# zj15001/PNP_ADMM_CNC_MRI

Measured on AMD Instinct MI355X. Metric: ADMM iterations/sec on 256x256 complex64 slices (batch=512), higher is better.
Workload: dtype f32

## Files before the change

### pnp_admm_cnc_mri_amd/csrc/api.hip

```cpp
#include "../../include/pnp_mri.h"
#include "internal.h"
#include "wavelet_plan.h"
#include "coil_plan.h"
#include "coilmix_plan.h"
#include "coilmaps_plan.h"

#include <math.h>
#include <stdarg.h>
#include <stdio.h>
#include <stdlib.h>
#include <string.h>
#include <dlfcn.h>
#include <new>
#include <type_traits>
#include <vector>

using namespace pnp;

static thread_local char g_err[512] = "";

int pnp::fail(int code, const char* fmt, ...) {
    va_list ap;
    va_start(ap, fmt);
    vsnprintf(g_err, sizeof(g_err), fmt, ap);
// ... 204 lines not shown
        if (c->mask_bank) { HIPCHK(hipStreamSynchronize(c->stream)); HIPCHK(hipFree(c->mask_bank)); c->mask_bank = nullptr; c->Kcap = 0; }
        HIPCHK(hipMalloc((void**)&c->mask_bank, (size_t)K * c->N));
        c->Kcap = K;
    }
    int rc = copy_in(c, c->mask_bank, mask_bank, (size_t)K * c->N, on_device);
    if (rc) return rc;
    if (mask_id) {
        std::vector<int32_t> tmp;
        const int32_t* ids = mask_id;
        if (on_device) {
            tmp.resize((size_t)B);
            HIPCHK(hipMemcpyAsync(tmp.data(), mask_id, (size_t)B * sizeof(int32_t), hipMemcpyDeviceToHost, c->stream));
            HIPCHK(hipStreamSynchronize(c->stream));
            ids = tmp.data();
        }
        for (int i = 0; i < B; ++i) if (ids[i] < 0 || ids[i] >= K) return fail(PNP_E_ARG, "mask_id[%d]=%d out of range [0,%d)", i, ids[i], K);
        rc = copy_in(c, c->mask_id, mask_id, (size_t)B * sizeof(int32_t), on_device);
        if (rc) return rc;
    } else {
        HIPCHK(hipMemsetAsync(c->mask_id, 0, (size_t)B * sizeof(int32_t), c->stream));
    }
    c->B = B; c->K = K;
    return PNP_OK;
}

static bool slice_pays(const pnp_ctx* c) { return c->B >= c->eng.slice_min_b; }

static int ensure_tables(pnp_ctx* c, Path path) {
    const float2* y = (const float2*)c->y;
    switch (path) {
    case Path::generic:
        return PNP_OK;
    case Path::slice:
        if (!c->prob.slice_built) HIPCHK(slice256_prepare(c->eng.slice, c->stream, y, c->mask_bank, c->mask_id, c->B));
        c->prob.slice_built = true;
        return PNP_OK;
    case Path::fused:
        if (c->prob.fused_built) return PNP_OK;
        switch (c->eng.kind) {
        case Engine::none:      return PNP_OK;
        case Engine::fused256:  HIPCHK(fused256_prepare(c->eng.f256, c->stream, y, c->mask_bank, c->mask_id, c->B)); break;
        case Engine::split_f32: HIPCHK(fused256s_prepare<float>(c->eng.s32, c->stream, c->y, c->mask_bank, c->mask_id, c->B)); break;
        case Engine::split_f64: HIPCHK(fused256s_prepare<double>(c->eng.s64, c->stream, c->y, c->mask_bank, c->mask_id, c->B)); break;
        case Engine::fused512:  HIPCHK(fused512_prepare(c->eng.f512, c->stream, y, c->mask_bank, c->mask_id, c->B)); break;
        }
        c->prob.fused_built = true;
        return PNP_OK;
    }
    return PNP_OK;
}

static int finish_problem(pnp_ctx* c, int rc) {
    if (rc == PNP_OK && c->eng.kind != Engine::none && c->coils.C == 0) {
        c->prob.path = (c->eng.slice && slice_pays(c)) ? Path::slice : Path::fused;
        if (c->prob.path == Path::fused) rc = ensure_tables(c, Path::fused);
    }
    if (rc != PNP_OK) { c->B = 0; c->prob = Problem{}; }
    return rc;
}

static Path loop_path(const pnp_ctx* c) { return (c->fast && c->coils.C == 0) ? c->prob.path : Path::generic; }
static Path dc_path(const pnp_ctx* c) { return loop_path(c) == Path::generic ? Path::generic : Path::fused; }

template <typename R> static int state_order(pnp_ctx* c, bool sliced) {
    if constexpr (std::is_same_v<R, double>) {
        return PNP_OK;
    } else {
// ... 1464 lines not shown
```

### pnp_admm_cnc_mri_amd/csrc/internal.h

```cpp
#pragma once
#include <hip/hip_runtime.h>
#include <stdint.h>
#include <stdlib.h>
#include "loop_schedule.h"
#include "prox_params.h"
#include "trace_plan.h"

namespace pnp {

int fail(int code, const char* fmt, ...) __attribute__((format(printf, 2, 3)));
#define HIPCHK(expr)                                                                               \
    do {                                                                                           \
        hipError_t _e = (expr);                                                                    \
        if (_e != hipSuccess)                                                                      \
            return fail(PNP_E_HIP, "%s failed: %s (%s:%d)", #expr, hipGetErrorString(_e), __FILE__, __LINE__); \
    } while (0)

template <typename R> struct CxOf;
template <> struct CxOf<float>  { using type = float2; };
template <> struct CxOf<double> { using type = double2; };

enum RowIn  { IN_COMPLEX = 0, IN_REAL = 1, IN_REAL_DIFF = 2 };
enum RowEpi { EPI_COMPLEX = 0, EPI_ABS_REAL = 1, EPI_ABS_COMPLEX = 2, EPI_L1 = 3, EPI_CNC = 4 };
enum ColMid { MID_NONE = 0, MID_BLEND = 1, MID_MASK = 2, MID_RESID = 3, MID_MASK_ADD = 4 };
// ... 135 lines not shown
hipError_t launch_conv3x3_tail_f16(hipStream_t s, const void* x_nhwc, const void* x2_nhwc , const float* w_oihw,
                                   const float* bias, float* y, int n, int cout, int H, int W, int shuffle_h = 0, int shuffle_w = 0);
hipError_t launch_pix2_pack_w_f16(hipStream_t s, const float* w, void* wfrag , int C, int up);
hipError_t launch_pix2x2_f16(hipStream_t s, const void* x, const void* x2, const void* wfrag, void* y, int n, int C, int H, int W, int up, int y_f32);

enum class ChainStep { open, cols, mid, last };

struct Fused256;
Fused256*  fused256_create(int Bmax, hipError_t* err);
void       fused256_destroy(Fused256*);
hipError_t fused256_prepare(Fused256*, hipStream_t s, const float2* y, const uint8_t* mask_bank,
                            const int32_t* mask_id, int B);
hipError_t fused256_run(Fused256*, hipStream_t s, float* z, float* w, float* x, int B, int iters,
                        bool cnc, float dc_c, ProxParams p, const FusedSchedule& sch);
hipError_t fused256_dc(Fused256*, hipStream_t s, const float* z, const float* w, float* x, int B, float dc_c);
hipError_t fused256_step(Fused256*, hipStream_t s, ChainStep st, const float* z, const float* w, float* zo, float* wo, float* x, int B,
                         bool cnc, float dc_c, ProxParams p, const FusedSchedule& sch, bool u_first);

template <typename R> struct Fused256S;
template <typename R> Fused256S<R>* fused256s_create(int Bmax, hipError_t* err);
template <typename R> void          fused256s_destroy(Fused256S<R>*);
template <typename R> hipError_t    fused256s_prepare(Fused256S<R>*, hipStream_t s, const void* y, const uint8_t* mask_bank,
                                                      const int32_t* mask_id, int B);
template <typename R> hipError_t    fused256s_run(Fused256S<R>*, hipStream_t s, R* z, R* w, R* x, int B, int iters, bool cnc,
                                                  R dc_c, ProxParamsT<R> p, const FusedSchedule& sch);
template <typename R> hipError_t    fused256s_dc(Fused256S<R>*, hipStream_t s, const R* z, const R* w, R* x, int B, R dc_c);
template <typename R> hipError_t    fused256s_step(Fused256S<R>*, hipStream_t s, ChainStep st, const R* z, const R* w, R* zo, R* wo, R* x, int B,
                                                   bool cnc, R dc_c, ProxParamsT<R> p, const FusedSchedule& sch, bool u_first);

struct Slice256;
Slice256*  slice256_create(int Bmax, int pad_kb , int yh_pad_kb , hipError_t* err);
void       slice256_destroy(Slice256*);
int        slice256_cus(const Slice256*);
hipError_t slice256_prepare(Slice256*, hipStream_t s, const float2* y, const uint8_t* mask_bank, const int32_t* mask_id, int B);
hipError_t slice256_run(Slice256*, hipStream_t s, float* z, float* w, float* x, int B, int iters, bool cnc, float dc_c,
                        ProxParams p, const FusedSchedule& sch);
hipError_t slice256_state_order(Slice256*, hipStream_t s, float* z, float* w, int B, bool to_slice);
hipError_t slice256_trace_snapshot(Slice256*, hipStream_t s, const float* z, int B);
hipError_t slice256_residuals(Slice256*, hipStream_t s, const float* x, const float* z, const float* w, const uint8_t* gt, int B,
                              double* partial, unsigned* counter, double* out);

struct Fused512;
Fused512*  fused512_create(int Bmax, hipError_t* err);
void       fused512_destroy(Fused512*);
hipError_t fused512_prepare(Fused512*, hipStream_t s, const float2* y, const uint8_t* mask_bank,
                            const int32_t* mask_id, int B);
hipError_t fused512_run(Fused512*, hipStream_t s, float* z, float* w, float* x, int B, int iters,
                        bool cnc, float dc_c, ProxParams p, const FusedSchedule& sch);
hipError_t fused512_dc(Fused512*, hipStream_t s, const float* z, const float* w, float* x, int B, float dc_c);
hipError_t fused512_step(Fused512*, hipStream_t s, ChainStep st, const float* z, const float* w, float* zo, float* wo, float* x, int B,
                         bool cnc, float dc_c, ProxParams p, const FusedSchedule& sch, bool u_first);

}
```

### pnp_admm_cnc_mri_amd/csrc/kernels_slice256.hip

```cpp
#include "engine_host.h"
#include "fused_layout.h"
#include "slice_layout.h"
#include <math.h>
#include <stdio.h>
#include <stdlib.h>
#include <vector>

#ifndef SLICE_EARLY
#define SLICE_EARLY 1
#endif
#ifndef SLICE_PRIOSWAP
#define SLICE_PRIOSWAP 1
#endif
#ifndef SLICE_PRIOMASK
#define SLICE_PRIOMASK 6
#endif
#ifndef SLICE_YH_AUX
#define SLICE_YH_AUX 0
#endif
#ifndef SLICE_ST_AUX
#define SLICE_ST_AUX 0
#endif
#ifndef SLICE_PF
#define SLICE_PF 3
#endif

namespace pnp {

__device__ c32 g_tws[256];

struct SliceArgs {
    float* z;
    float* w;
    float* x;
    const c32* Yh;
    const uint32_t* Mh;
    const c32* Ys;
    const uint32_t* Ms;
    int first, B, iters;
    int slice_xor;
    int flip;
    int state_stride;
    int yh_stride;
    float scale, c;
    ProxParams prox;
    long long* prof;
};

constexpr int RP = 18;
constexpr int REGION = 16 * RP;
constexpr int WREG = 4 * REGION;
constexpr int SL_YS = SL_BUF + REGION;
constexpr int SL_LDS = SL_YS + 256 + 32;
static_assert(SL_WAVES * WREG <= SL_BUF, "wave regions must fit in the buffer they alias");
__device__ __forceinline__ int sl_lds_float(int set, int q) { return set == 0 ? sl_res_index(0, 0, q) : sl_res1_index(popc8(sl_units_lds(set) & ((1u << q) - 1)), 0, 0); }
static_assert(REGION * 8 == SL2_TW_BYTES && (256 + 32) * 8 == SL2_YS_BYTES && SL2_END % 8 == 0, "tables of the LDS map");
template <int PROX> constexpr bool slice_four() { return PROX == 2; }
template <int PROX> constexpr bool slice_res() { return slice_four<PROX>() && SLICE_RESIDENT; }
__device__ __forceinline__ void lds_ld4(const float* p, float (&v)[4]) {
    const float4 q = *reinterpret_cast<const float4*>(p);
    v[0] = q.x; v[1] = q.y; v[2] = q.z; v[3] = q.w;
}
__device__ __forceinline__ void lds_st4(float* p, const float (&v)[4]) { *reinterpret_cast<float4*>(p) = make_float4(v[0], v[1], v[2], v[3]); }

__device__ __forceinline__ void wave_sync() {
    __builtin_amdgcn_fence(__ATOMIC_RELEASE, "wavefront");
    __builtin_amdgcn_wave_barrier();
    __builtin_amdgcn_fence(__ATOMIC_ACQUIRE, "wavefront");
#ifdef SLICE_SYNC_SCHED_BARRIER
    __builtin_amdgcn_sched_barrier(0);
#endif
// ... 265 lines not shown
    const int voff = 2048 * g + 16 * t;
    float* const resl[2] = {RES ? res_lane(res, 0, wv, lane) : nullptr, RES && SL_NLDS1 ? res_lane(res, 1, wv, lane) : nullptr};
    constexpr bool RES_LOOP = RES && HAS_INV;
    constexpr int PF = row_pf<PROX>();
    RowLoads L;
    if (PRELOADED) L = *pre;
    else issue_row_loads<PROX, HAS_INV, 0, PF, RES_LOOP>(b, L, row_set_offset(0, wv), voff, 0, 0, resl[0]);
#pragma unroll
    for (int set = 0; set < SL_SETS; ++set) {
        c32 (&a)[16] = F[set];
        prio_set(wv, set);
        const int soff = row_set_offset(set, wv);
        if (HAS_INV) {
            group_fft256<true, SPLIT>(a, twl, region, t);
        }
        if (HAS_INV && last) store_x_natural<SPLIT>(b, a, wreg, set, wv, lane);
        const int vs = voff + soff;
#pragma unroll
        for (int q = 0; q < 8; ++q) {
            const int home = RES ? w_home(set, q) : W_HBM;
            float* const rl = home == W_LDS ? resl[set] + sl_lds_float(set, q) : nullptr;
            float* const wq = wr[home == W_REG ? sl_reg_slot(set, q) : 0];
            if (q + PF < 8) issue_row_loads<PROX, HAS_INV, 0, 1, RES_LOOP>(b, L, soff, voff, q + PF, set, resl[set < 2 ? set : 0]);
            if (RES_LOOP && home != W_HBM) {
                pointwise_q<HAS_INV, PROX, HAS_FWD>(b, pc, u_first, last, a[2 * q], a[2 * q + 1], L.z[q], home == W_REG ? wr[sl_reg_slot(set, q)] : L.w[q],
                                                    vs + ROW_QSTRIDE * q, home, rl, wq);
            } else {
                if (home == W_LDS) lds_st4(rl, L.w[q]);
                if (home == W_REG) { wq[0] = L.w[q][0]; wq[1] = L.w[q][1]; wq[2] = L.w[q][2]; wq[3] = L.w[q][3]; }
                pointwise_q<HAS_INV, PROX, HAS_FWD>(b, pc, u_first, last, a[2 * q], a[2 * q + 1], L.z[q], L.w[q], vs + ROW_QSTRIDE * q);
            }
        }
        if (set + 1 < SL_SETS) issue_row_loads<PROX, HAS_INV, 0, PF, RES_LOOP>(b, L, row_set_offset(set + 1, wv), voff, 0, set + 1, resl[set + 1 < 2 ? set + 1 : 0]);
        if (HAS_FWD) {
            group_fft256<false, SPLIT>(a, twl, region, t);
        }
    }
}

__device__ __forceinline__ void resident_flush(const SliceBufs& b, float* res, const ResRegs& wr, int wv, int lane) {
#pragma unroll
    for (int set = 0; set < SL_SETS; ++set) {
        const int vs = 2048 * (lane >> 4) + 16 * (lane & 15) + row_set_offset(set, wv);
#pragma unroll
        for (int q = 0; q < 8; ++q) {
            const int home = w_home(set, q);
            if (home == W_LDS) {
                float v[4];
                lds_ld4(res_lane(res, set, wv, lane) + sl_lds_float(set, q), v);
                st4(b.w, vs + ROW_QSTRIDE * q, 0, v);
            } else if (home == W_REG) {
                st4(b.w, vs + ROW_QSTRIDE * q, 0, wr[sl_reg_slot(set, q)]);
            }
        }
    }
}

#define SL_PASS0_REGS(X, t)                                                                       \
    X(0, 0, (t)) X(1, 1, (t) + 16) X(2, 2, (t) + 32) X(3, 3, (t) + 48)                              \
    X(12, 8, ((t) ? SL_M + 64 - (t) : SL_M))                                                      \
    X(13, 13, SL_M + 48 - (t)) X(14, 14, SL_M + 32 - (t)) X(15, 15, SL_M + 16 - (t))
#define SL_PASS1_REGS(X, t)                                                                       \
    X(4, 4, (t)) X(5, 5, (t) + 16) X(6, 6, (t) + 32) X(7, 7, (t) + 48)                              \
    X(8, 12, ((t) ? SL_M + 64 - (t) : SL_M))                                                      \
    X(9, 9, SL_M + 48 - (t)) X(10, 10, SL_M + 32 - (t)) X(11, 11, SL_M + 16 - (t))

#define SL_PASS4_REGS(X, t, Q)                                                                    \
// ... 196 lines not shown
        prio_set(wv, set);
        group_fft256<false, SPLIT>(a, twl, region, t);
        if (set == 0 && wv == 0 && g == 0) {
#pragma unroll
            for (int j = 0; j < 16; ++j) region[t + 16 * j] = a[j];
            region[256 + t] = a[0];
            wave_sync();
            const uint32_t code_b = reinterpret_cast<const uint32_t*>(ysl + 256)[t];
            const c32* mirror = region + (16 - t);
            const unsigned ma[4] = {Y.code & 0x03030303u, (Y.code >> 2) & 0x03030303u, (Y.code >> 4) & 0x03030303u, (Y.code >> 6) & 0x03030303u};
            const unsigned mb[4] = {code_b & 0x03030303u, (code_b >> 2) & 0x03030303u, (code_b >> 4) & 0x03030303u, (code_b >> 6) & 0x03030303u};
#pragma unroll
            for (int j = 0; j < 16; ++j) {
                const c32 gm = mirror[16 * (15 - j)];
                const c32 A = blend_scaled_f(unpack_a(a[j], gm), Y.yh[j], code_byte(ma[j & 3], j >> 2), cs, chs, scale);
                const c32 Bv = blend_scaled_f(unpack_b(a[j], gm), ysl[t + 16 * j], code_byte(mb[j & 3], j >> 2), cs, chs, scale);
                a[j] = repack_p(A, Bv);
            }
            wave_sync();
        } else {
            blend_set(a, Y.yh, Y.code, cs, 0.5f * chs, 0.5f * scale);
        }
        if (set + 1 < SL_SETS) issue_col_loads(b, Y, set + 1, wv, lane);
        group_fft256<true, SPLIT>(a, twl, region, t);
    }
}

template <int PROX>
__global__ __launch_bounds__(512) void k_slice(SliceArgs p) {
    constexpr bool FOUR = slice_four<PROX>(), RES = slice_res<PROX>();
    __shared__ __attribute__((aligned(16))) c32 lds[FOUR ? SL2_END / 8 : SL_LDS];
    const int tid = threadIdx.x, lane = tid & 63;
    const int wv = __builtin_amdgcn_readfirstlane(tid >> 6);
    c32* twl = lds + (FOUR ? SL2_TW / 8 : SL_BUF);
    c32* ysl = lds + (FOUR ? SL2_YS / 8 : SL_YS);
    float* res = RES ? reinterpret_cast<float*>(lds + SL2_RES0 / 8) : nullptr;
    if (tid < 256) twl[RP * (tid >> 4) + (tid & 15)] = g_tws[((tid >> 4) * (tid & 15)) & 255];
    c32* wreg = FOUR ? reinterpret_cast<c32*>(reinterpret_cast<float*>(lds) + wv * SL_XWAVE) : lds + wv * WREG;
    __syncthreads();
    for (int sb = blockIdx.x; sb < p.B; sb += gridDim.x) {
        const int sx = ((sb ^ p.slice_xor) < p.B) ? (sb ^ p.slice_xor) : sb;
        const int slice = p.first + (p.flip ? p.B - 1 - sx : sx);
        const size_t so = (size_t)slice * p.state_stride;
        SliceBufs b;
        b.z = make_rsrc(p.z + so, 65536 * 4); b.w = make_rsrc(p.w + so, 65536 * 4); b.x = make_rsrc(p.x + (size_t)slice * 65536, 65536 * 4);
        b.yh = make_rsrc(p.Yh + (size_t)slice * p.yh_stride, YH3_SLICE * 8); b.mh = make_rsrc(p.Mh + (size_t)slice * MH3_SLICE, MH3_SLICE * 4);
        b.ys = make_rsrc(p.Ys + (size_t)slice * 256, 256 * 8); b.ms = make_rsrc(p.Ms + (size_t)slice * 16, 16 * 4);
        c32 F[SL_SETS][16];
        ResRegs wres;
#ifdef SLICE_PROF
        long long* prof = (p.prof && tid == 0 && sb == (int)blockIdx.x) ? p.prof + (size_t)slice * (2 + 6 * p.iters) : nullptr;
#define SL_STAMP() if (prof) *prof++ = wall_clock64()
#else
#define SL_STAMP()
#endif
        SL_STAMP();
        row_phase<false, 0, true, false, RES, FOUR>(b, p.prox, 1, false, F, wreg, twl, wv, opaque(lane), wres, nullptr, res);
        SL_STAMP();
        for (int it = 0; it < p.iters; ++it) {
            c32 G[SL_SETS][16];
            __syncthreads();
            SL_STAMP();
            if (FOUR) {
                t1_pass8<0>(F, G, lds, wv, opaque(lane));
                t1_pass8<1>(F, G, lds, wv, opaque(lane));
                t1_pass8<2>(F, G, lds, wv, opaque(lane));
                t1_pass8<3>(F, G, lds, wv, opaque(lane));
            } else {
                t1_pass<0>(F, G, lds, wv, opaque(lane));
                t1_pass<1>(F, G, lds, wv, opaque(lane));
            }
#ifdef SLICE_PROF_CLOCK
            if (prof) *prof++ = (long long)__builtin_readcyclecounter();
#else
            SL_STAMP();
#endif
            col_phase<FOUR>(b, p.c, p.scale, G, wreg, ysl, twl, wv, opaque(lane));
            SL_STAMP();
            __syncthreads();
            SL_STAMP();
            if (FOUR) {
                t2_pass8<0>(G, F, lds, wv, opaque(lane));
                t2_pass8<1>(G, F, lds, wv, opaque(lane));
                t2_pass8<2>(G, F, lds, wv, opaque(lane));
            } else {
                t2_pass<0>(G, F, lds, wv, opaque(lane));
            }
#if SLICE_EARLY
            RowLoads L0;
            row_phase_prefetch<PROX, true, RES>(b, L0, wv, opaque(lane), res);
#endif
            if (FOUR) t2_pass8<3>(G, F, lds, wv, opaque(lane));
            else t2_pass<1>(G, F, lds, wv, opaque(lane));
            SL_STAMP();
            const int u_first = (it == 0);
#if SLICE_EARLY
            row_phase<true, PROX, true, true, RES, FOUR>(b, p.prox, u_first, it + 1 == p.iters, F, wreg, twl, wv, opaque(lane), wres, &L0, res);
#else
            row_phase<true, PROX, true, false, RES, FOUR>(b, p.prox, u_first, it + 1 == p.iters, F, wreg, twl, wv, opaque(lane), wres, nullptr, res);
#endif
            SL_STAMP();
        }
        if (RES) resident_flush(b, res, wres, wv, opaque(lane));
        __syncthreads();
    }
}

constexpr int SP_P = 17;
__global__ __launch_bounds__(256) void k_sprepare(const c32* y, const uint8_t* mask_bank, const int32_t* mask_id,
                                                  c32* Yh, uint32_t* Mh, c32* Ys, uint32_t* Ms, int yh_stride) {
    __shared__ c32 yd[256 * SP_P], ym[256 * SP_P];
    __shared__ uint8_t md[256 * SP_P], mm[256 * SP_P];
    const int tid = threadIdx.x, m = blockIdx.x, slice = blockIdx.y;
    const int mid = mask_id ? mask_id[slice] : 0;
    const c32* ys = y + (size_t)slice * 65536;
    const uint8_t* ms = mask_bank + (size_t)mid * 65536;
    const int ncol = (m == 8) ? 1 : 16;
#pragma unroll 4
    for (int i = 0; i < 16; ++i) {
        const int idx = tid + 256 * i, r = idx >> 4, c = idx & 15;
        if (c < ncol) {
            const int k2 = 16 * m + c, k2m = (256 - k2) & 255;
            yd[r * SP_P + c] = ys[r * 256 + k2];
            md[r * SP_P + c] = ms[r * 256 + k2];
            ym[r * SP_P + c] = ys[r * 256 + k2m];
            mm[r * SP_P + c] = ms[r * 256 + k2m];
        }
    }
    __syncthreads();
    auto entry = [&](int k1, int c, c32& yh) -> int {
        const int r2 = (256 - k1) & 255;
        const int m1 = md[k1 * SP_P + c] != 0, m2 = mm[r2 * SP_P + c] != 0;
        const c32 y1 = yd[k1 * SP_P + c], y2 = ym[r2 * SP_P + c];
        yh = mk<float>(0.5f * ((m1 ? y1.x : 0.f) + (m2 ? y2.x : 0.f)), 0.5f * ((m1 ? y1.y : 0.f) - (m2 ? y2.y : 0.f)));
        return m1 + m2;
    };
    if (m == 8) {
        c32 yh;
        const int code = entry(tid, 0, yh);
        Ys[(size_t)slice * 256 + tid] = yh;
        __shared__ int codes[256];
        codes[tid] = code;
        __syncthreads();
        if (tid < 16) {
            uint32_t v = 0;
#pragma unroll
            for (int jj = 0; jj < 16; ++jj) v |= (uint32_t)codes[tid + 16 * jj] << (2 * jj);
            Ms[slice * 16 + tid] = v;
        }
        return;
    }
    const int set = m >> 1;
#pragma unroll 4
    for (int i = 0; i < 16; ++i) {
        const int o = tid + 256 * i, blk = o >> 10, e = o & 1023;
        const int jp = e >> 7, lane = (e >> 1) & 63, j = 2 * jp + (e & 1);
        const int g = lane >> 4, t = lane & 15, wv = 4 * (m & 1) + blk;
        c32 yh;
        (void)entry(t + 16 * j, 4 * blk + g, yh);
        Yh[(size_t)slice * yh_stride + yh3_index(0, set, j, wv, lane)] = yh;
    }
    {
        const int blk = tid >> 6, lane = tid & 63, g = lane >> 4, t = lane & 15, wv = 4 * (m & 1) + blk;
        uint32_t v = 0;
#pragma unroll
        for (int j = 0; j < 16; ++j) {
            c32 yh;
            v |= (uint32_t)entry(t + 16 * j, 4 * blk + g, yh) << (2 * j);
        }
        Mh[mh3_index(slice, set, wv, lane)] = v;
    }
}

template <bool TO_SLICE>
__global__ __launch_bounds__(128) void k_state_order(const float* sz, const float* sw, float* dz, float* dw, int src_stride, int dst_stride) {
    __shared__ float tile[2][2048];
    const size_t sbase = (size_t)blockIdx.y * src_stride + (size_t)blockIdx.x * 2048, dbase = (size_t)blockIdx.y * dst_stride + (size_t)blockIdx.x * 2048;
    const float4* pz = reinterpret_cast<const float4*>(sz + sbase);
    const float4* pw = reinterpret_cast<const float4*>(sw + sbase);
    float4* qz = reinterpret_cast<float4*>(dz + dbase);
    float4* qw = reinterpret_cast<float4*>(dw + dbase);
    float4 vz[4], vw[4];
#pragma unroll
    for (int u = 0; u < 4; ++u) { vz[u] = pz[threadIdx.x + 128 * u]; vw[u] = pw[threadIdx.x + 128 * u]; }
#pragma unroll
    for (int u = 0; u < 4; ++u) {
        const int i = threadIdx.x + 128 * u, row = i >> 6, n0 = 4 * (i & 63);
        const float az[4] = {vz[u].x, vz[u].y, vz[u].z, vz[u].w}, aw[4] = {vw[u].x, vw[u].y, vw[u].z, vw[u].w};
#pragma unroll
        for (int k = 0; k < 4; ++k) {
            const int at = TO_SLICE ? (int)sl_state_index(row, n0 + k) : 4 * i + k;
            tile[0][at] = az[k];
            tile[1][at] = aw[k];
        }
    }
    __syncthreads();
#pragma unroll
    for (int u = 0; u < 4; ++u) {
        const int i = threadIdx.x + 128 * u, row = i >> 6, n0 = 4 * (i & 63);
        float oz[4], ow[4];
#pragma unroll
        for (int k = 0; k < 4; ++k) {
            const int at = TO_SLICE ? 4 * i + k : (int)sl_state_index(row, n0 + k);
            oz[k] = tile[0][at];
            ow[k] = tile[1][at];
        }
        qz[i] = make_float4(oz[0], oz[1], oz[2], oz[3]);
        qw[i] = make_float4(ow[0], ow[1], ow[2], ow[3]);
    }
}

struct Slice256 {
    int Bmax = 0, cus = 0;
    int flip = 0;
    int pad = 0, yh_pad = 0;
    float* zs = nullptr;
    float* ws = nullptr;
    float* zprev = nullptr;
    c32* Yh = nullptr;
    uint32_t* Mh = nullptr;
    c32* Ys = nullptr;
    uint32_t* Ms = nullptr;
    SideQueues queues;
};

int slice256_cus(const Slice256* f) { return f && f->cus > 0 ? f->cus : 256; }

hipError_t slice256_state_order(Slice256* f, hipStream_t s, float* z, float* w, int B, bool to_slice) {
    if (B <= 0) return hipSuccess;
    if (f && f->pad > 0) {
        if (to_slice) hipLaunchKernelGGL(k_state_order<true>, dim3(32, B), dim3(128), 0, s, z, w, f->zs, f->ws, 65536, 65536 + f->pad);
        else          hipLaunchKernelGGL(k_state_order<false>, dim3(32, B), dim3(128), 0, s, f->zs, f->ws, z, w, 65536 + f->pad, 65536);
    } else {
        if (to_slice) hipLaunchKernelGGL(k_state_order<true>, dim3(32, B), dim3(128), 0, s, z, w, z, w, 65536, 65536);
        else          hipLaunchKernelGGL(k_state_order<false>, dim3(32, B), dim3(128), 0, s, z, w, z, w, 65536, 65536);
    }
    return hipGetLastError();
}

hipError_t slice256_trace_snapshot(Slice256* f, hipStream_t s, const float* z, int B) {
    const size_t stride = 65536 + (size_t)f->pad;
    if (B > f->Bmax) return hipErrorInvalidValue;
    if (!f->zprev) { hipError_t e = hipMalloc((void**)&f->zprev, (size_t)f->Bmax * stride * sizeof(float)); if (e != hipSuccess) return e; }
    return hipMemcpyAsync(f->zprev, f->pad > 0 ? f->zs : z, (size_t)B * stride * sizeof(float), hipMemcpyDeviceToDevice, s);
}
hipError_t slice256_residuals(Slice256* f, hipStream_t s, const float* x, const float* z, const float* w, const uint8_t* gt, int B,
                              double* partial, unsigned* counter, double* out) {
    if (!f->zprev || B > f->Bmax) return hipErrorInvalidValue;
    return launch_residuals<float>(s, x, f->pad > 0 ? f->zs : z, f->zprev, f->pad > 0 ? f->ws : w, gt, 0, B, 65536, 65536 + (size_t)f->pad, true,
                                   partial, counter, out);
}

void slice256_destroy(Slice256* f) {
    if (!f) return;
    if (f->zs) (void)hipFree(f->zs);
    if (f->ws) (void)hipFree(f->ws);
    if (f->zprev) (void)hipFree(f->zprev);
    if (f->Yh) (void)hipFree(f->Yh);
    if (f->Mh) (void)hipFree(f->Mh);
    if (f->Ys) (void)hipFree(f->Ys);
    if (f->Ms) (void)hipFree(f->Ms);
    delete f;
}

Slice256* slice256_create(int Bmax, int pad_kb, int yh_pad_kb, hipError_t* err) {
    Slice256* f = new Slice256();
    f->Bmax = Bmax;
    f->pad = (pad_kb > 0 ? pad_kb : 0) * 256;
    f->yh_pad = (yh_pad_kb > 0 ? yh_pad_kb : 0) * 128;
    hipError_t e = hipMalloc((void**)&f->Yh, (size_t)Bmax * (YH3_SLICE + f->yh_pad) * sizeof(c32));
    if (e == hipSuccess && f->pad > 0) e = hipMalloc((void**)&f->zs, (size_t)Bmax * (65536 + f->pad) * sizeof(float));
    if (e == hipSuccess && f->pad > 0) e = hipMalloc((void**)&f->ws, (size_t)Bmax * (65536 + f->pad) * sizeof(float));
    if (e == hipSuccess) e = hipMalloc((void**)&f->Mh, (size_t)Bmax * MH3_SLICE * sizeof(uint32_t));
    if (e == hipSuccess) e = hipMalloc((void**)&f->Ys, (size_t)Bmax * 256 * sizeof(c32));
    if (e == hipSuccess) e = hipMalloc((void**)&f->Ms, (size_t)Bmax * 16 * sizeof(uint32_t));
    if (e == hipSuccess) e = upload_twiddle_table<float>(HIP_SYMBOL(g_tws), 256);
    if (e == hipSuccess) {
        int dev = 0;
        hipDeviceProp_t prop;
        e = hipGetDevice(&dev);
        if (e == hipSuccess) e = hipGetDeviceProperties(&prop, dev);
        if (e == hipSuccess) f->cus = prop.multiProcessorCount;
    }
    if (e != hipSuccess) {
        slice256_destroy(f);
        *err = e;
        return nullptr;
    }
    *err = hipSuccess;
    return f;
}

hipError_t slice256_prepare(Slice256* f, hipStream_t s, const float2* y, const uint8_t* mask_bank, const int32_t* mask_id, int B) {
    if (B > f->Bmax) return hipErrorInvalidValue;
    hipLaunchKernelGGL(k_sprepare, dim3(9, B), dim3(256), 0, s, reinterpret_cast<const c32*>(y), mask_bank, mask_id,
                       f->Yh, f->Mh, f->Ys, f->Ms, (int)YH3_SLICE + f->yh_pad);
    return hipGetLastError();
}

static hipError_t launch_slice(hipStream_t s, const SliceArgs& a, int prox) {
    const dim3 grid(a.B);
    if (prox == 2)      hipLaunchKernelGGL(k_slice<2>, grid, dim3(512), 0, s, a);
    else if (prox == 1) hipLaunchKernelGGL(k_slice<1>, grid, dim3(512), 0, s, a);
    else                hipLaunchKernelGGL(k_slice<3>, grid, dim3(512), 0, s, a);
    return hipGetLastError();
}

hipError_t slice256_run(Slice256* f, hipStream_t s, float* z, float* w, float* x, int B, int iters, bool cnc, float dc_c,
                        ProxParams pp, const FusedSchedule& sch) {
    if (iters <= 0) return hipSuccess;
    SliceArgs a;
    a.z = f->pad > 0 ? f->zs : z; a.w = f->pad > 0 ? f->ws : w; a.x = x; a.Yh = f->Yh;
    a.state_stride = 65536 + f->pad; a.yh_stride = (int)YH3_SLICE + f->yh_pad; a.Mh = f->Mh; a.Ys = f->Ys; a.Ms = f->Ms;
    a.first = 0; a.B = B; a.iters = iters; a.scale = 1.0f / 65536.0f; a.c = dc_c;
    a.prox = pp;
    a.prof = nullptr;
    a.flip = 0;
    a.slice_xor = sch.slice_xor;
    if (a.slice_xor < 0 || (B & (B - 1)) != 0 || a.slice_xor >= B) a.slice_xor = 0;
    const int prox = prox_kind(cnc, sch);
    int segments = sch.slice_segment > 0 ? (iters + sch.slice_segment - 1) / sch.slice_segment : 1;
    if (segments < 1) segments = 1;

    long long* d_prof = nullptr;
#ifdef SLICE_PROF
    const char* prof_path = getenv("PNP_SLICE_PROF");
#else
    const char* prof_path = nullptr;
#endif
    const LoopPlan plan = plan_slice(B, prof_path ? FusedSchedule{} : sch);
    const size_t prof_n = (size_t)B * (2 + 6 * (size_t)iters);
    if (prof_path) {
        segments = 1;
        if (hipMalloc((void**)&d_prof, prof_n * sizeof(long long)) == hipSuccess) {
            (void)hipMemsetAsync(d_prof, 0, prof_n * sizeof(long long), s);
            a.prof = d_prof;
        }
    }
    if (!prof_path && B > slice256_cus(f) && sch.slice_flip) { a.flip = f->flip; f->flip ^= 1; }
    const hipError_t e = run_parts(f->queues, s, plan, B, [&](hipStream_t sq, const Part& p) {
        hipError_t r = hipSuccess;
        int done = 0;
        for (int g = 0; g < segments && r == hipSuccess; ++g) {
            const int n = (iters - done + (segments - g) - 1) / (segments - g);
            a.first = p.first; a.B = p.count; a.iters = n;
            r = launch_slice(sq, a, prox);
            done += n;
        }
        return r;
    });
    if (d_prof) {
        std::vector<long long> h(prof_n);
        (void)hipStreamSynchronize(s);
        (void)hipMemcpy(h.data(), d_prof, prof_n * sizeof(long long), hipMemcpyDeviceToHost);
        (void)hipFree(d_prof);
        if (FILE* fo = fopen(prof_path, "wb")) {
            const int hdr[2] = {B, iters};
            fwrite(hdr, sizeof(int), 2, fo);
            fwrite(h.data(), sizeof(long long), prof_n, fo);
            fclose(fo);
        }
    }
    return e;
}

}
```

### pnp_admm_cnc_mri_amd/csrc/loop_schedule.h

```cpp
#pragma once

namespace pnp {

constexpr int kMaxQueues = 4;

struct FusedSchedule {
    int queues = 2;
    int mixed = 0;
    int chunk = 0;
    int l1_two_state = 0;
    int chunk_queues = 0;
    int slice_xor = 0;
    int slice_queues = 1;
    int slice_segment = 0;
    int slice_flip = 1;
};

inline int prox_kind(bool cnc, const FusedSchedule& sch) { return cnc ? 2 : (sch.l1_two_state ? 1 : 3); }

struct LoopPlan {
    int queues;
    int chunk;
    int launches;
    bool mixed;
// ... 16 lines not shown
            return {1, chunk, 2 * n, false, n, chunk};
        }
        return {1, B, 2, false, 1, B};
    }
    if (queues >= 2 && B >= 32 * queues) return {queues, B, 2 * queues, sch.mixed != 0, queues, ((B / queues) + 1) & ~1};
    return {1, B, 2, queues == 1 && sch.mixed != 0, 1, B};
}

enum class Chunked { split_f32, split_f64, fused512 };
inline LoopPlan plan_chunked(int B, const FusedSchedule& sch, Chunked kind) {
    const bool is512 = kind == Chunked::fused512;
    int queues = sch.chunk_queues > 0 ? sch.chunk_queues : (sch.queues >= 2 ? 4 : 1);
    if (queues > kMaxQueues) queues = kMaxQueues;
    const int dflt = is512 ? (queues >= 2 ? 16 : 48) : (kind == Chunked::split_f64 ? (queues >= 2 ? 24 : 96) : 0);
    int chunk = sch.chunk != 0 ? sch.chunk : dflt;
    if (chunk <= 0) {
        if (!is512 && sch.queues >= 2 && B >= 64) { queues = 2; chunk = ((B / 2) + 1) & ~1; }
        else { queues = 1; chunk = B; }
    }
    chunk &= ~1;
    if (chunk < 2) chunk = 2;
    if (chunk >= B) { chunk = B > 2 ? ((B + 1) & ~1) : 2; queues = 1; }
    const int n = (B + chunk - 1) / chunk;
    const int part = chunk < B ? chunk : B;
    return {queues, part, 2 * n, false, n, part};
}

inline LoopPlan plan_slice(int B, const FusedSchedule& sch) {
    int queues = sch.slice_queues < 1 ? 1 : (sch.slice_queues > kMaxQueues ? kMaxQueues : sch.slice_queues);
    if (B < 64 * queues) queues = 1;
    return {queues, B, 0, false, queues, B / queues};
}

}
```

### profiles/micro/slice_stride.hip

```cpp
#include <hip/hip_runtime.h>
#include <algorithm>
#include <cstdio>
#include <cstdlib>
#include <vector>
#define CK(x) do { hipError_t e_ = (x); if (e_ != hipSuccess) { fprintf(stderr, "%s: %s\n", #x, hipGetErrorString(e_)); exit(1); } } while (0)

__global__ __launch_bounds__(512) void k_slices(float4* z, float4* w, const float4* y, size_t stride16, int iters, int pause_ticks, long long* t, int who, int throttle, int res_acc) {
    if ((who == 1 && !(blockIdx.x & 1)) || (who == 2 && (blockIdx.x & 1))) { if (threadIdx.x == 0) t[blockIdx.x] = 0; return; }
    const size_t base = (size_t)blockIdx.x * stride16;
    float4* zs = z + base;
    float4* ws = w + base;
    const float4* ys = y + base;
    const int tid = threadIdx.x;
    const long long t0 = wall_clock64();
    for (int it = 0; it < iters; ++it) {
        for (int g = 0; g < 4; ++g) {
            float4 a[8], b[8], c[8];
#pragma unroll
            for (int u = 0; u < 8; ++u) { const int i = tid + 512 * (8 * g + u); a[u] = zs[i]; b[u] = (8 * g + u < res_acc) ? make_float4(0.f, 0.f, 0.f, 0.f) : ws[i]; c[u] = ys[i]; }
#pragma unroll
            for (int u = 0; u < 8; ++u) {
                const int i = tid + 512 * (8 * g + u);
                zs[i] = make_float4(a[u].x + c[u].x * 1e-9f, a[u].y + c[u].y * 1e-9f, a[u].z + c[u].z * 1e-9f, a[u].w + c[u].w * 1e-9f);
                if (8 * g + u >= res_acc) ws[i] = make_float4(b[u].x - c[u].x * 1e-9f, b[u].y - c[u].y * 1e-9f, b[u].z - c[u].z * 1e-9f, b[u].w - c[u].w * 1e-9f);
            }
        }
        if (throttle > 0 && !(blockIdx.x & 1)) for (int k = 0; k < throttle; ++k) __builtin_amdgcn_s_sleep(24);
        if (pause_ticks > 0) {
            const long long p0 = wall_clock64();
            while (wall_clock64() - p0 < pause_ticks) __builtin_amdgcn_s_sleep(8);
        }
    }
    if (tid == 0) t[blockIdx.x] = wall_clock64() - t0;
}

int main(int argc, char** argv) {
    const size_t pad_kib = argc > 1 ? (size_t)atoi(argv[1]) : 0;
    const int slices = argc > 2 ? atoi(argv[2]) : 256;
    const int iters = argc > 3 ? atoi(argv[3]) : 50;
    const int pause_us = argc > 4 ? atoi(argv[4]) : 0;
    const int who = argc > 5 ? atoi(argv[5]) : 0, throttle = argc > 6 ? atoi(argv[6]) : 0;
    const int resident = argc > 7 ? atoi(argv[7]) : 0, pause_tenths = argc > 8 ? atoi(argv[8]) : 0;
    const size_t stride = (256 + pad_kib) << 10, bytes = stride * slices;
    float4 *z, *w, *y; long long* t;
    CK(hipMalloc(&z, bytes)); CK(hipMalloc(&w, bytes)); CK(hipMalloc(&y, bytes)); CK(hipMalloc(&t, slices * sizeof(long long)));
    CK(hipMemset(z, 0, bytes)); CK(hipMemset(w, 0, bytes)); CK(hipMemset(y, 0, bytes));
    hipEvent_t e0, e1; CK(hipEventCreate(&e0)); CK(hipEventCreate(&e1));
    std::vector<long long> h(slices);
    for (int rep = 0; rep < 3; ++rep) {
        CK(hipEventRecord(e0));
        hipLaunchKernelGGL(k_slices, dim3(slices), dim3(512), 0, 0, z, w, y, stride / 16, iters, pause_us * 100 + pause_tenths * 10, t, who, throttle, resident / 4);
        CK(hipEventRecord(e1)); CK(hipEventSynchronize(e1));
        float ms; CK(hipEventElapsedTime(&ms, e0, e1));
        CK(hipMemcpy(h.data(), t, slices * sizeof(long long), hipMemcpyDeviceToHost));
        std::vector<double> ev, od;
        for (int b = 0; b < slices; ++b) ((b & 1) ? od : ev).push_back(h[b] / 100.0 / iters);
        std::sort(ev.begin(), ev.end()); std::sort(od.begin(), od.end());
        const double moved = (5.0 * 262144.0 - 2.0 * 2048.0 * (resident / 4 * 4)) * (who ? slices / 2 : slices) * iters;
        printf("{\"resident\": %d, \"pause_extra_tenths\": %d, \"who\": %d, \"throttle\": %d, \"pad_KiB\": %zu, \"slices\": %d, \"iters\": %d, \"pause_us\": %d, \"rep\": %d, \"ms\": %.3f, \"TBps\": %.3f, "
               "\"us_per_iteration_even_median\": %.2f, \"us_per_iteration_odd_median\": %.2f, \"even_max\": %.2f, \"odd_max\": %.2f}\n",
               resident, pause_tenths, who, throttle, pad_kib, slices, iters, pause_us, rep, ms, moved / (ms * 1e-3) / 1e12,
               ev[ev.size() / 2], od[od.size() / 2], ev.back(), od.back());
    }
    return 0;
}
```

Baseline: 11930.

## Share mask tables per mask id instead of per slice in slice256 path

Mask-derived tables (Mh, Ms) are now built once per distinct mask id (K) and indexed through mask_id in the slice kernel, instead of being replicated per slice. This is meant to shrink the mask footprint and the cache pressure from per-slice mask reads. The prepare step is split into two launches, and the mask buffers are reallocated lazily with a stream sync. It also adds start-stagger and skip-last-forward-FFT options, which are disabled by default, plus profiling scripts.

```diff
diff --git a/pnp_admm_cnc_mri_amd/csrc/api.hip b/pnp_admm_cnc_mri_amd/csrc/api.hip
--- a/pnp_admm_cnc_mri_amd/csrc/api.hip
+++ b/pnp_admm_cnc_mri_amd/csrc/api.hip
@@ -260,7 +260,7 @@
     case Path::generic:
         return PNP_OK;
     case Path::slice:
-        if (!c->prob.slice_built) HIPCHK(slice256_prepare(c->eng.slice, c->stream, y, c->mask_bank, c->mask_id, c->B));
+        if (!c->prob.slice_built) HIPCHK(slice256_prepare(c->eng.slice, c->stream, y, c->mask_bank, c->mask_id, c->B, c->K));
         c->prob.slice_built = true;
         return PNP_OK;
     case Path::fused:
diff --git a/pnp_admm_cnc_mri_amd/csrc/internal.h b/pnp_admm_cnc_mri_amd/csrc/internal.h
--- a/pnp_admm_cnc_mri_amd/csrc/internal.h
+++ b/pnp_admm_cnc_mri_amd/csrc/internal.h
@@ -191,7 +191,7 @@
 Slice256*  slice256_create(int Bmax, int pad_kb , int yh_pad_kb , hipError_t* err);
 void       slice256_destroy(Slice256*);
 int        slice256_cus(const Slice256*);
-hipError_t slice256_prepare(Slice256*, hipStream_t s, const float2* y, const uint8_t* mask_bank, const int32_t* mask_id, int B);
+hipError_t slice256_prepare(Slice256*, hipStream_t s, const float2* y, const uint8_t* mask_bank, const int32_t* mask_id, int B, int K);
 hipError_t slice256_run(Slice256*, hipStream_t s, float* z, float* w, float* x, int B, int iters, bool cnc, float dc_c,
                         ProxParams p, const FusedSchedule& sch);
 hipError_t slice256_state_order(Slice256*, hipStream_t s, float* z, float* w, int B, bool to_slice);
diff --git a/pnp_admm_cnc_mri_amd/csrc/kernels_slice256.hip b/pnp_admm_cnc_mri_amd/csrc/kernels_slice256.hip
--- a/pnp_admm_cnc_mri_amd/csrc/kernels_slice256.hip
+++ b/pnp_admm_cnc_mri_amd/csrc/kernels_slice256.hip
@@ -20,6 +20,21 @@
 #endif
 #ifndef SLICE_ST_AUX
 #define SLICE_ST_AUX 0
+#endif
+#ifndef SLICE_SKIP_LAST_FWD
+#define SLICE_SKIP_LAST_FWD 0
+#endif
+#ifndef SLICE_MASK_SHARED
+#define SLICE_MASK_SHARED 1
+#endif
+#ifndef SLICE_STAGGER
+#define SLICE_STAGGER 0
+#endif
+#ifndef SLICE_STAGGER_CLASS
+#define SLICE_STAGGER_CLASS 0
+#endif
+#ifndef SLICE_STAGGER_US
+#define SLICE_STAGGER_US 20
 #endif
 #ifndef SLICE_PF
 #define SLICE_PF 3
@@ -37,6 +52,8 @@
     const uint32_t* Mh;
     const c32* Ys;
     const uint32_t* Ms;
+    const int32_t* mask_id;
+    int cus, stagger;
     int first, B, iters;
     int slice_xor;
     int flip;
@@ -368,7 +385,8 @@
             }
         }
         if (set + 1 < SL_SETS) issue_row_loads<PROX, HAS_INV, 0, PF, RES_LOOP>(b, L, row_set_offset(set + 1, wv), voff, 0, set + 1, resl[set + 1 < 2 ? set + 1 : 0]);
-        if (HAS_FWD) {
+        constexpr bool SKIP = HAS_INV && (SLICE_SKIP_LAST_FWD == 2 || (SLICE_SKIP_LAST_FWD == 1 && PROX == 2));
+        if (HAS_FWD && !(SKIP && last)) {
             group_fft256<false, SPLIT>(a, twl, region, t);
         }
     }
@@ -631,6 +649,15 @@
     __shared__ __attribute__((aligned(16))) c32 lds[FOUR ? SL2_END / 8 : SL_LDS];
     const int tid = threadIdx.x, lane = tid & 63;
     const int wv = __builtin_amdgcn_readfirstlane(tid >> 6);
+#if SLICE_STAGGER
+    if (PROX == 2) {
+        const int ticks = stagger_block(p.stagger, p.cus, SLICE_STAGGER_CLASS, (int)blockIdx.x);
+        if (ticks > 0) {
+            const long long t0 = wall_clock64();
+            for (int i = 0; i < kStaggerSpins && wall_clock64() - t0 < ticks; ++i) __builtin_amdgcn_s_sleep(4);
+        }
+    }
+#endif
     c32* twl = lds + (FOUR ? SL2_TW / 8 : SL_BUF);
     c32* ysl = lds + (FOUR ? SL2_YS / 8 : SL_YS);
     float* res = RES ? reinterpret_cast<float*>(lds + SL2_RES0 / 8) : nullptr;
@@ -643,8 +670,9 @@
         const size_t so = (size_t)slice * p.state_stride;
         SliceBufs b;
         b.z = make_rsrc(p.z + so, 65536 * 4); b.w = make_rsrc(p.w + so, 65536 * 4); b.x = make_rsrc(p.x + (size_t)slice * 65536, 65536 * 4);
-        b.yh = make_rsrc(p.Yh + (size_t)slice * p.yh_stride, YH3_SLICE * 8); b.mh = make_rsrc(p.Mh + (size_t)slice * MH3_SLICE, MH3_SLICE * 4);
-        b.ys = make_rsrc(p.Ys + (size_t)slice * 256, 256 * 8); b.ms = make_rsrc(p.Ms + (size_t)slice * 16, 16 * 4);
+        b.yh = make_rsrc(p.Yh + (size_t)slice * p.yh_stride, YH3_SLICE * 8); const int mcode = SLICE_MASK_SHARED ? (p.mask_id ? p.mask_id[slice] : 0) : slice;
+        b.mh = make_rsrc(p.Mh + mh3_index(mcode, 0, 0, 0), MH3_SLICE * 4);
+        b.ys = make_rsrc(p.Ys + (size_t)slice * 256, 256 * 8); b.ms = make_rsrc(p.Ms + (size_t)mcode * 16, 16 * 4);
         c32 F[SL_SETS][16];
         ResRegs wres;
 #ifdef SLICE_PROF
@@ -706,13 +734,14 @@
 }
 
 constexpr int SP_P = 17;
+template <bool CODES>
 __global__ __launch_bounds__(256) void k_sprepare(const c32* y, const uint8_t* mask_bank, const int32_t* mask_id,
                                                   c32* Yh, uint32_t* Mh, c32* Ys, uint32_t* Ms, int yh_stride) {
     __shared__ c32 yd[256 * SP_P], ym[256 * SP_P];
     __shared__ uint8_t md[256 * SP_P], mm[256 * SP_P];
     const int tid = threadIdx.x, m = blockIdx.x, slice = blockIdx.y;
-    const int mid = mask_id ? mask_id[slice] : 0;
-    const c32* ys = y + (size_t)slice * 65536;
+    const int mid = (CODES && SLICE_MASK_SHARED) ? slice : (mask_id ? mask_id[slice] : 0);
+    const c32* ys = y + (size_t)(CODES ? 0 : slice) * 65536;
     const uint8_t* ms = mask_bank + (size_t)mid * 65536;
     const int ncol = (m == 8) ? 1 : 16;
 #pragma unroll 4
@@ -737,7 +766,7 @@
     if (m == 8) {
         c32 yh;
         const int code = entry(tid, 0, yh);
-        Ys[(size_t)slice * 256 + tid] = yh;
+        if (!CODES) { Ys[(size_t)slice * 256 + tid] = yh; return; }
         __shared__ int codes[256];
         codes[tid] = code;
         __syncthreads();
@@ -751,7 +780,7 @@
     }
     const int set = m >> 1;
 #pragma unroll 4
-    for (int i = 0; i < 16; ++i) {
+    for (int i = 0; i < (CODES ? 0 : 16); ++i) {
         const int o = tid + 256 * i, blk = o >> 10, e = o & 1023;
         const int jp = e >> 7, lane = (e >> 1) & 63, j = 2 * jp + (e & 1);
         const int g = lane >> 4, t = lane & 15, wv = 4 * (m & 1) + blk;
@@ -759,7 +788,7 @@
         (void)entry(t + 16 * j, 4 * blk + g, yh);
         Yh[(size_t)slice * yh_stride + yh3_index(0, set, j, wv, lane)] = yh;
     }
-    {
+    if (CODES) {
         const int blk = tid >> 6, lane = tid & 63, g = lane >> 4, t = lane & 15, wv = 4 * (m & 1) + blk;
         uint32_t v = 0;
 #pragma unroll
@@ -811,6 +840,8 @@
 
 struct Slice256 {
     int Bmax = 0, cus = 0;
+    int codes = 0;
+    const int32_t* mask_id = nullptr;
     int flip = 0;
     int pad = 0, yh_pad = 0;
     float* zs = nullptr;
@@ -870,9 +901,7 @@
     hipError_t e = hipMalloc((void**)&f->Yh, (size_t)Bmax * (YH3_SLICE + f->yh_pad) * sizeof(c32));
     if (e == hipSuccess && f->pad > 0) e = hipMalloc((void**)&f->zs, (size_t)Bmax * (65536 + f->pad) * sizeof(float));
     if (e == hipSuccess && f->pad > 0) e = hipMalloc((void**)&f->ws, (size_t)Bmax * (65536 + f->pad) * sizeof(float));
-    if (e == hipSuccess) e = hipMalloc((void**)&f->Mh, (size_t)Bmax * MH3_SLICE * sizeof(uint32_t));
     if (e == hipSuccess) e = hipMalloc((void**)&f->Ys, (size_t)Bmax * 256 * sizeof(c32));
-    if (e == hipSuccess) e = hipMalloc((void**)&f->Ms, (size_t)Bmax * 16 * sizeof(uint32_t));
     if (e == hipSuccess) e = upload_twiddle_table<float>(HIP_SYMBOL(g_tws), 256);
     if (e == hipSuccess) {
         int dev = 0;
@@ -890,9 +919,25 @@
     return f;
 }
 
-hipError_t slice256_prepare(Slice256* f, hipStream_t s, const float2* y, const uint8_t* mask_bank, const int32_t* mask_id, int B) {
-    if (B > f->Bmax) return hipErrorInvalidValue;
-    hipLaunchKernelGGL(k_sprepare, dim3(9, B), dim3(256), 0, s, reinterpret_cast<const c32*>(y), mask_bank, mask_id,
+hipError_t slice256_prepare(Slice256* f, hipStream_t s, const float2* y, const uint8_t* mask_bank, const int32_t* mask_id, int B, int K) {
+    if (B > f->Bmax || K < 1) return hipErrorInvalidValue;
+    const int codes = SLICE_MASK_SHARED ? K : B;
+    if (codes > f->codes) {
+        const int room = SLICE_MASK_SHARED ? K : f->Bmax;
+        hipError_t e = hipStreamSynchronize(s);
+        if (e != hipSuccess) return e;
+        if (f->Mh) (void)hipFree(f->Mh);
+        if (f->Ms) (void)hipFree(f->Ms);
+        f->Mh = nullptr; f->Ms = nullptr; f->codes = 0;
+        e = hipMalloc((void**)&f->Mh, (size_t)room * MH3_SLICE * sizeof(uint32_t));
+        if (e == hipSuccess) e = hipMalloc((void**)&f->Ms, (size_t)room * 16 * sizeof(uint32_t));
+        if (e != hipSuccess) return e;
+        f->codes = room;
+    }
+    f->mask_id = mask_id;
+    hipLaunchKernelGGL(k_sprepare<false>, dim3(9, B), dim3(256), 0, s, reinterpret_cast<const c32*>(y), mask_bank, mask_id,
+                       f->Yh, f->Mh, f->Ys, f->Ms, (int)YH3_SLICE + f->yh_pad);
+    hipLaunchKernelGGL(k_sprepare<true>, dim3(9, codes), dim3(256), 0, s, reinterpret_cast<const c32*>(y), mask_bank, mask_id,
                        f->Yh, f->Mh, f->Ys, f->Ms, (int)YH3_SLICE + f->yh_pad);
     return hipGetLastError();
 }
@@ -915,6 +960,8 @@
     a.prox = pp;
     a.prof = nullptr;
     a.flip = 0;
+    a.mask_id = f->mask_id;
+    a.cus = slice256_cus(f); a.stagger = 0;
     a.slice_xor = sch.slice_xor;
     if (a.slice_xor < 0 || (B & (B - 1)) != 0 || a.slice_xor >= B) a.slice_xor = 0;
     const int prox = prox_kind(cnc, sch);
@@ -937,6 +984,9 @@
         }
     }
     if (!prof_path && B > slice256_cus(f) && sch.slice_flip) { a.flip = f->flip; f->flip ^= 1; }
+#if SLICE_STAGGER
+    if (!prof_path && prox == 2 && plan.parts == 1) a.stagger = plan_stagger(B, a.cus, iters / segments, SLICE_STAGGER_US * kStaggerTicksPerUs);
+#endif
     const hipError_t e = run_parts(f->queues, s, plan, B, [&](hipStream_t sq, const Part& p) {
         hipError_t r = hipSuccess;
         int done = 0;
diff --git a/pnp_admm_cnc_mri_amd/csrc/loop_schedule.h b/pnp_admm_cnc_mri_amd/csrc/loop_schedule.h
--- a/pnp_admm_cnc_mri_amd/csrc/loop_schedule.h
+++ b/pnp_admm_cnc_mri_amd/csrc/loop_schedule.h
@@ -72,4 +72,24 @@
     return {queues, B, 0, false, queues, B / queues};
 }
 
+constexpr int kStaggerTicksPerUs = 100;
+constexpr int kStaggerSlackPerIter = 330;
+constexpr int kStaggerSlackMax = 51 * kStaggerTicksPerUs;
+constexpr int kStaggerMaxTicks = kStaggerSlackMax / 4;
+constexpr int kStaggerSpins = 4096;
+constexpr int stagger_cap(int K) {
+    const long long slack = (long long)(K > 0 ? K : 0) * kStaggerSlackPerIter;
+    return (int)((slack > kStaggerSlackMax ? kStaggerSlackMax : slack) / 4);
 }
+constexpr int plan_stagger(int B, int cus, int K, int wait) {
+    if (cus < 1 || B <= cus || wait <= 0) return 0;
+    return wait < stagger_cap(K) ? wait : stagger_cap(K);
+}
+constexpr int stagger_block(int launch_wait, int cus, int slack_class, int block) {
+    return (block < cus && (block & 1) == slack_class) ? launch_wait : 0;
+}
+constexpr int stagger_wait(int B, int cus, int K, int wait, int slack_class, int block) {
+    return stagger_block(plan_stagger(B, cus, K, wait), cus, slack_class, block);
+}
+
+}
diff --git a/profiles/launch_ends.py b/profiles/launch_ends.py
--- /dev/null
+++ b/profiles/launch_ends.py
@@ -0,0 +1,47 @@
+#!/usr/bin/env python3
+import sys
+import numpy as np
+raw = open(sys.argv[1], 'rb').read()
+B, iters = (int(v) for v in np.frombuffer(raw[:8], np.int32))
+cus = int(sys.argv[2]) if len(sys.argv) > 2 else 256
+t = np.frombuffer(raw[8:], np.int64).reshape(B, 2 + 6 * iters).astype(np.float64) / 100.0
+t0 = t[:, 0].min()
+start, end = t[:, 0] - t0, t[:, -1] - t0
+dur = end - start
+first = t[:, 1] - t[:, 0]
+ph = t[:, 2:].reshape(B, iters, 6)
+prev = np.concatenate([t[:, 1:2], ph[:, :-1, 5]], axis=1)
+it = ph[:, :, 5] - prev
+rows = ph[:, :, 5] - ph[:, :, 4]
+idx = np.arange(B)
+rounds = [('round 1', idx < cus)] + ([('round 2', idx >= cus)] if B > cus else [])
+makespan = end.max()
+print('slices %d, iterations %d, compute units %d: makespan %.1f us = %.2f us per batched iteration' % (B, iters, cus, makespan, makespan / iters))
+print('idle share: 1 - sum of workgroup durations / (units x makespan) = %.2f %%' % (100 * (1 - dur.sum() / min(cus, B) / makespan)))
+steady = np.median(it[:, min(8, iters - 1):]) if iters > 8 else np.median(it)
+print('steady iteration (median over workgroups, iterations 9..): %.2f us;  2 rounds x K x steady = %.1f us = %.1f %% of the makespan' % (
+    steady, 2 * iters * steady, 100 * 2 * iters * steady / makespan))
+for name, sel in rounds:
+    print(name)
+    print('  XCD  blocks  start(med)  end(med)  end(max)  rows(first)  iterations 1..6 (median, us)                 steady   rows(steady)')
+    for x in range(8):
+        s = sel & (idx % 8 == x)
+        if not s.any():
+            continue
+        k = min(6, iters)
+        st = np.median(it[s][:, min(8, iters - 1):]) if iters > 8 else np.median(it[s])
+        rs = np.median(rows[s][:, min(8, iters - 1):]) if iters > 8 else np.median(rows[s])
+        print('  %d    %4d    %8.1f  %8.1f  %8.1f   %8.2f     %s   %6.2f   %6.2f' % (
+            x, s.sum(), np.median(start[s]), np.median(end[s]), end[s].max(), np.median(first[s]),
+            ' '.join('%6.1f' % v for v in np.median(it[s][:, :k], axis=0)), st, rs))
+    for par in (0, 1):
+        s = sel & ((idx & 1) == par)
+        if s.any():
+            k = min(6, iters)
+            st = np.median(it[s][:, min(8, iters - 1):]) if iters > 8 else np.median(it[s])
+            extra = float(np.sum(np.median(it[s][:, :k], axis=0) - st))
+            print('  %s blocks: end median %.1f max %.1f;  rows(first) %.2f;  iterations 1..%d cost %.1f us more than %d steady ones' % (
+                'odd ' if par else 'even', np.median(end[s]), end[s].max(), np.median(first[s]), k, extra, k))
+ev, od = end[(idx & 1) == 0].max(), end[(idx & 1) == 1].max()
+print('slack of the class that ends first: even blocks end by %.1f us, odd blocks by %.1f us -> %.1f us (%s class waits)' % (
+    ev, od, abs(od - ev), 'even' if ev < od else 'odd'))
diff --git a/profiles/micro/slice_stride.hip b/profiles/micro/slice_stride.hip
--- a/profiles/micro/slice_stride.hip
+++ b/profiles/micro/slice_stride.hip
@@ -5,13 +5,17 @@
 #include <vector>
 #define CK(x) do { hipError_t e_ = (x); if (e_ != hipSuccess) { fprintf(stderr, "%s: %s\n", #x, hipGetErrorString(e_)); exit(1); } } while (0)
 
-__global__ __launch_bounds__(512) void k_slices(float4* z, float4* w, const float4* y, size_t stride16, int iters, int pause_ticks, long long* t, int who, int throttle, int res_acc) {
+__global__ __launch_bounds__(512) void k_slices(float4* z, float4* w, const float4* y, size_t stride16, int iters, int pause_ticks, long long* t, int who, int throttle, int res_acc, int start_ticks, int start_parity) {
     if ((who == 1 && !(blockIdx.x & 1)) || (who == 2 && (blockIdx.x & 1))) { if (threadIdx.x == 0) t[blockIdx.x] = 0; return; }
     const size_t base = (size_t)blockIdx.x * stride16;
     float4* zs = z + base;
     float4* ws = w + base;
     const float4* ys = y + base;
     const int tid = threadIdx.x;
+    if (start_ticks > 0 && (int)(blockIdx.x & 1) == start_parity) {
+        const long long s0 = wall_clock64();
+        for (int k = 0; k < 4096 && wall_clock64() - s0 < start_ticks; ++k) __builtin_amdgcn_s_sleep(4);
+    }
     const long long t0 = wall_clock64();
     for (int it = 0; it < iters; ++it) {
         for (int g = 0; g < 4; ++g) {
@@ -41,6 +45,7 @@
     const int pause_us = argc > 4 ? atoi(argv[4]) : 0;
     const int who = argc > 5 ? atoi(argv[5]) : 0, throttle = argc > 6 ? atoi(argv[6]) : 0;
     const int resident = argc > 7 ? atoi(argv[7]) : 0, pause_tenths = argc > 8 ? atoi(argv[8]) : 0;
+    const int start_us = argc > 9 ? atoi(argv[9]) : 0, start_parity = argc > 10 ? atoi(argv[10]) & 1 : 0;
     const size_t stride = (256 + pad_kib) << 10, bytes = stride * slices;
     float4 *z, *w, *y; long long* t;
     CK(hipMalloc(&z, bytes)); CK(hipMalloc(&w, bytes)); CK(hipMalloc(&y, bytes)); CK(hipMalloc(&t, slices * sizeof(long long)));
@@ -49,7 +54,8 @@
     std::vector<long long> h(slices);
     for (int rep = 0; rep < 3; ++rep) {
         CK(hipEventRecord(e0));
-        hipLaunchKernelGGL(k_slices, dim3(slices), dim3(512), 0, 0, z, w, y, stride / 16, iters, pause_us * 100 + pause_tenths * 10, t, who, throttle, resident / 4);
+        hipLaunchKernelGGL(k_slices, dim3(slices), dim3(512), 0, 0, z, w, y, stride / 16, iters, pause_us * 100 + pause_tenths * 10, t, who, throttle, resident / 4,
+                           std::min(start_us, 1000) * 100, start_parity);
         CK(hipEventRecord(e1)); CK(hipEventSynchronize(e1));
         float ms; CK(hipEventElapsedTime(&ms, e0, e1));
         CK(hipMemcpy(h.data(), t, slices * sizeof(long long), hipMemcpyDeviceToHost));
@@ -57,9 +63,9 @@
         for (int b = 0; b < slices; ++b) ((b & 1) ? od : ev).push_back(h[b] / 100.0 / iters);
         std::sort(ev.begin(), ev.end()); std::sort(od.begin(), od.end());
         const double moved = (5.0 * 262144.0 - 2.0 * 2048.0 * (resident / 4 * 4)) * (who ? slices / 2 : slices) * iters;
-        printf("{\"resident\": %d, \"pause_extra_tenths\": %d, \"who\": %d, \"throttle\": %d, \"pad_KiB\": %zu, \"slices\": %d, \"iters\": %d, \"pause_us\": %d, \"rep\": %d, \"ms\": %.3f, \"TBps\": %.3f, "
+        printf("{\"start_offset_us\": %d, \"start_parity\": %d, \"resident\": %d, \"pause_extra_tenths\": %d, \"who\": %d, \"throttle\": %d, \"pad_KiB\": %zu, \"slices\": %d, \"iters\": %d, \"pause_us\": %d, \"rep\": %d, \"ms\": %.3f, \"TBps\": %.3f, "
                "\"us_per_iteration_even_median\": %.2f, \"us_per_iteration_odd_median\": %.2f, \"even_max\": %.2f, \"odd_max\": %.2f}\n",
-               resident, pause_tenths, who, throttle, pad_kib, slices, iters, pause_us, rep, ms, moved / (ms * 1e-3) / 1e12,
+               start_us, start_parity, resident, pause_tenths, who, throttle, pad_kib, slices, iters, pause_us, rep, ms, moved / (ms * 1e-3) / 1e12,
                ev[ev.size() / 2], od[od.size() / 2], ev.back(), od.back());
     }
     return 0;
```

Result: faster. 12100, median of 6 (+1.4%).
